# tier4/icp_rust

Hardware: AMD Instinct MI355X
Metric: ICP iterations/sec on 1M-pt 3D pair (higher is better)
Workload: dtype f64

## Files before the change

icp_rust_amd/csrc/nn_grid.hip:

```cpp
#include "common.hpp"
#include <type_traits>

namespace icp {

__device__ __forceinline__ int cell_coord(double v, double lo, double inv_h, int n) {
  double t = floor((v - lo) * inv_h);
  t = fmin(fmax(t, 0.), (double)(n - 1));
  return (int)t;
}

__global__ void k_grid_bbox(const double *__restrict__ dst, unsigned m, int dim, double *__restrict__ part) {
  __shared__ double smn[3][256], smx[3][256];
  double mn[3], mx[3];
  for (int d = 0; d < 3; ++d) {
    mn[d] = __builtin_huge_val();
    mx[d] = -__builtin_huge_val();
  }
  for (unsigned i = blockIdx.x * 256 + threadIdx.x; i < m; i += gridDim.x * 256)
    for (int d = 0; d < dim; ++d) {
      const double v = dst[(size_t)i * dim + d];
      mn[d] = fmin(mn[d], v);
      mx[d] = fmax(mx[d], v);
    }
  for (int d = 0; d < 3; ++d) {
// ... 799 lines not shown
    }
  };

  int iz = lo_c[2], iy = lo_c[1];
  float dz2 = (DIM == 3 && !wide) ? slab2(2, iz) : 0.f;
  for (;;) {
    uint32_t ra0 = 0, ra1 = 0, ra2 = 0, ra3 = 0, rz0 = 0, rz1 = 0, rz2 = 0, rz3 = 0;
    int nr = 0;
    while (nr < 4 && iz <= hi_c[2]) {
      if (iy > hi_c[1]) {
        iy = lo_c[1];
        ++iz;
        if (DIM == 3 && !wide && iz <= hi_c[2]) dz2 = slab2(2, iz);
        continue;
      }
      const int cy = iy++;
      int xl = lo_c[0], xh = hi_c[0];
      if (!wide) {
        const float dyz = slab2(1, cy) + dz2;
        if (dyz > bf) {
          if (CERT) skip2 = fminf(skip2, dyz);
          continue;
        }
        const float hw = __builtin_amdgcn_sqrtf(bf - dyz) * 1.000001f + mgf;
        xl = max(xl, cell_lo(qf[0] - hw, em[0], 0));
        xh = min(xh, cell_hi(qf[0] + hw, em[0], 0));
        if (xl > xh) {
          if (CERT) skip2 = 0.f;
          continue;
        }
        if (CERT) {
          if (xl > lo_c[0]) skip2 = fminf(skip2, slab2(0, xl - 1) + dyz);
          if (xh < hi_c[0]) skip2 = fminf(skip2, slab2(0, xh + 1) + dyz);
        }
      }
      const uint32_t rb = ((uint32_t)iz * g.n[1] + cy) * g.n[0];
      const uint32_t ra = rb + xl, rz = rb + xh + 1;
      if (nr == 0) ra0 = ra, rz0 = rz;
      else if (nr == 1) ra1 = ra, rz1 = rz;
      else if (nr == 2) ra2 = ra, rz2 = rz;
      else ra3 = ra, rz3 = rz;
      ++nr;
    }
    if (nr == 0) break;
    if (nr < 2) ra1 = ra0, rz1 = rz0;
    if (nr < 3) ra2 = ra0, rz2 = rz0;
    if (nr < 4) ra3 = ra0, rz3 = rz0;
    const uint32_t s0 = start[ra0], e0 = start[rz0];
    const uint32_t s1 = start[ra1], e1 = start[rz1];
    const uint32_t s2 = start[ra2], e2 = start[rz2];
    const uint32_t s3 = start[ra3], e3 = start[rz3];
    const uint32_t n0 = e0 > s0 ? (e0 - s0 + 3) >> 2 : 0u;
    const uint32_t n1 = (nr > 1 && e1 > s1) ? (e1 - s1 + 3) >> 2 : 0u;
    const uint32_t n2 = (nr > 2 && e2 > s2) ? (e2 - s2 + 3) >> 2 : 0u;
    const uint32_t n3 = (nr > 3 && e3 > s3) ? (e3 - s3 + 3) >> 2 : 0u;
    const uint32_t o1 = n0, o2 = o1 + n1, o3 = o2 + n2, Q = o3 + n3;
    const uint32_t d0 = s0, d1 = s1 - 4u * o1, d2 = s2 - 4u * o2, d3 = s3 - 4u * o3;
    constexpr uint32_t kQ = ICP_WARM_QUADS, kR = 4 * kQ;
    for (uint32_t base = 0; base < Q; base += kQ) {
      GridPoint t[kR];
      const uint4 *line[kQ];
#pragma unroll
      for (uint32_t h2 = 0; h2 < kQ; ++h2) {
        const uint32_t j = min(base + h2, Q - 1);
        uint32_t dq = d0;
        if (j >= o1) dq = d1;
        if (j >= o2) dq = d2;
        if (j >= o3) dq = d3;
        line[h2] = reinterpret_cast<const uint4 *>(pts) + (size_t)(uint32_t)(4u * j + dq);
      }
#pragma unroll
      for (uint32_t u = 0; u < kR; ++u) {
        const uint4 w = line[u >> 2][u & 3];
        t[u].x = __uint_as_float(w.x);
        t[u].y = __uint_as_float(w.y);
        t[u].z = __uint_as_float(w.z);
        t[u].idx = w.w;
      }
      __builtin_amdgcn_sched_barrier(0);
      float sc[kR];
#pragma unroll
      for (uint32_t u = 0; u < kR; ++u) {
        const float fx = qf[0] - t[u].x, fy = qf[1] - t[u].y;
        float s2 = __builtin_fmaf(fy, fy, fx * fx);
        if (DIM == 3) {
          const float fz = qf[2] - t[u].z;
          s2 = __builtin_fmaf(fz, fz, s2);
        }
        sc[u] = s2;
      }
#pragma unroll
      for (uint32_t u = 0; u < kR; ++u)
        if (!(sc[u] > thr32) && t[u].idx != bi) consider(t[u].idx);
      if (CERT) {
#pragma unroll
        for (uint32_t u = 0; u < kR; ++u) m2 = fminf(m2, t[u].idx != bi ? sc[u] : __builtin_huge_valf());
      }
    }
  }
  uint32_t cert_bits = 0;
  if (CERT && !wide && bi != 0xffffffffu) {
    const float seen = __builtin_amdgcn_sqrtf(m2) * 0.9999994f - ecf;
    const float skipped = __builtin_amdgcn_sqrtf(skip2) * 0.9999997f;
    const float cert = fminf(seen, skipped);
    const float abs_lo = (cert + (cd.r_lo * s_norm_lo + cd.t_lo) * 0.9999997f) * 0.9999997f;
    if (cert > 0.f && abs_lo > 0.f && abs_lo < __builtin_huge_valf()) cert_bits = __float_as_uint(abs_lo);
  }
  if (bi == 0xffffffffu) {
    bi = 0;
    bx = dst[0];
    by = dst[1];
    bz = DIM == 3 ? dst[2] : 0.;
  }
  if (CERT || SEEDED || bi != pm.idx) {
    PrevMatch out;
    out.x = bx;
    out.y = by;
    out.z = bz;
    out.idx = bi;
    out.pad = cert_bits;
    prev[k] = out;
  }
  if (idx) idx[i] = bi;
  if (a) a[i] = make_double2(q[0], q[1]);
  if (b) b[i] = make_double2(bx, by);
}

template <int DIM, bool CERT>
__global__ __launch_bounds__(kGridThreads) ICP_WARM_ATTR void k_nn_grid_warm(const double *__restrict__ src,
                                                               const uint32_t *__restrict__ perm, unsigned n, Pose T,
                                                               GridParams g, const uint32_t *__restrict__ start,
                                                               const GridPoint *__restrict__ pts,
                                                               const double *__restrict__ dst, uint32_t *__restrict__ idx,
                                                               double2 *__restrict__ a, double2 *__restrict__ b,
                                                               PrevMatch *prev, CertDecay cd, unsigned xcd_chunk) {
  const unsigned k = xcd_wave(blockIdx.x, gridDim.x, xcd_chunk) * kGridThreads + threadIdx.x;
  if (k >= n) return;
  warm_query<DIM, CERT>(k, src, perm, T, g, start, pts, dst, idx, a, b, prev, cd);
}

#ifndef ICP_COOP_ITEMS
#define ICP_COOP_ITEMS 2
#endif
#ifndef ICP_COOP_ROWS
#define ICP_COOP_ROWS 4
#endif
#ifndef ICP_COOP_FLUSH_AT
#define ICP_COOP_FLUSH_AT 96
#endif
constexpr int kCoopItems = ICP_COOP_ITEMS;
constexpr int kCoopRows = ICP_COOP_ROWS;
constexpr int kCoopCandCap = 256;
constexpr int kCoopFlushAt = ICP_COOP_FLUSH_AT;
struct CoopLds {
  uint32_t pref[64];
  uint32_t rows_d[64][kCoopRows];
  uint32_t rows_o[64][kCoopRows];
  float4 oq[64];
  uint32_t obi[64];
  uint2 cand[kCoopCandCap];
  unsigned long long fkey[64];
  uint32_t fidx[64];
  uint32_t fwin[64];
};

#ifdef ICP_COOP_PROFILE
__device__ unsigned long long g_coop_prof[64][12];
__device__ long long g_coop_span[16384][2];
__device__ unsigned long long g_coop_rows[32];
#define COOP_STAMP(i)                                                  \
  do {                                                                 \
    asm volatile("s_waitcnt vmcnt(0) lgkmcnt(0)" ::: "memory");        \
    const long long now_ = wall_clock64();                             \
    cprof[i] += (unsigned long long)(now_ - ct_last);                  \
    ct_last = now_;                                                    \
  } while (0)
#define COOP_COUNT(i, v) (cprof[i] += (v))
#else
#define COOP_STAMP(i) ((void)0)
#define COOP_COUNT(i, v) ((void)0)
#endif

template <int DIM, bool SEEDED>
__device__ __forceinline__ void warm_wave(const unsigned k, const unsigned n, const double *__restrict__ src,
                                          const uint32_t *__restrict__ perm, Pose T, const GridParams &g,
                                          const uint32_t *__restrict__ start, const GridPoint *__restrict__ pts,
                                          const double *__restrict__ dst, uint32_t *__restrict__ idx,
                                          double2 *__restrict__ a, double2 *__restrict__ b, PrevMatch *prev, PrevMatch seed,
                                          CoopLds &S) {
  const unsigned lane = threadIdx.x;
#ifdef ICP_COOP_PROFILE
  unsigned long long cprof[12] = {0, 0, 0, 0, 0, 0, 0, 1, 0, 0, 0, 0};
  long long ct_last = wall_clock64();
  const long long ct_first = ct_last;
#endif
  const bool in_range = k < n;
  const unsigned kk = in_range ? k : n - 1;
  const unsigned i = perm ? perm[kk] : kk;
  double q[3];
  q[0] = src[(size_t)kk * DIM + 0];
  q[1] = src[(size_t)kk * DIM + 1];
  q[2] = DIM == 3 ? src[(size_t)kk * DIM + 2] : 0.;
  {
    const double nx = (T.r00 * q[0] + T.r01 * q[1]) + T.tx;
    const double ny = (T.r10 * q[0] + T.r11 * q[1]) + T.ty;
    q[0] = nx;
    q[1] = ny;
  }
  const PrevMatch pm = SEEDED ? seed : prev[kk];
  const bool no_match = pm.idx == 0xffffffffu;
  bool alive = in_range && !no_match;
  auto dist2 = [&](double tx, double ty, double tz) -> double {
    const double ddx = q[0] - tx, ddy = q[1] - ty;
    double dd = ddx * ddx + ddy * ddy;
    if (DIM == 3) {
      const double ddz = q[2] - tz;
      dd = dd + ddz * ddz;
    }
    return dd;
  };
  double best = dist2(pm.x, pm.y, pm.z);
  uint32_t bi = pm.idx;
  double bx = pm.x, by = pm.y, bz = pm.z;
  if (!(best == best)) {
    best = __builtin_huge_val();
    bi = 0xffffffffu;
  }
  float qf[3], amax = 0.f;
#pragma unroll
  for (int d = 0; d < 3; ++d) {
    qf[d] = d < DIM ? (float)(q[d] - g.lo[d]) : 0.f;
    amax = fmaxf(amax, fabsf(qf[d]));
  }
  const float mgf = 4e-7f * (amax + g.ext);
  const float ecf = 2.1e-7f * (amax + g.ext);
  float bf, rf, thr32;
  auto set_radius = [&]() {
    bf = fmaxf((float)best * 1.0000003f, 1e-37f);
    const float rs = __builtin_amdgcn_sqrtf(bf) * 1.0000003f;
    rf = rs + mgf;
    thr32 = (rs + ecf) * (rs + ecf) * 1.000005f;
  };
  set_radius();
  const bool wide = !(amax + rf < 1e18f);
  if (wide) {
    bf = __builtin_huge_valf();
    thr32 = __builtin_huge_valf();
  }
  const float hf[3] = {g.hf[0], g.hf[1], g.hf[2]};
  const float ihf[3] = {g.ihf[0], g.ihf[1], g.ihf[2]};
  auto cell_lo = [&](float v, float em, int d) -> int {
    const float t = fminf(fmaxf(__builtin_floorf(v * ihf[d] - em), 0.f), g.nm1f[d]);
    return (int)t;
  };
  auto cell_hi = [&](float v, float em, int d) -> int {
    const float t = fminf(fmaxf(__builtin_floorf(v * ihf[d] + em), 0.f), g.nm1f[d]);
    return (int)t;
  };
  int lo_c[3] = {0, 0, 0}, hi_c[3] = {0, 0, 0};
  float em[3];
#pragma unroll
  for (int d = 0; d < DIM; ++d) {
    em[d] = (fabsf(qf[d]) + rf) * ihf[d] * 4e-7f + 1e-3f;
    lo_c[d] = wide ? 0 : cell_lo(qf[d] - rf, em[d], d);
    hi_c[d] = wide ? g.n[d] - 1 : cell_hi(qf[d] + rf, em[d], d);
  }
  auto slab2 = [&](int d, int c) -> float {
    const float e0 = (float)c * hf[d];
    const float below = c <= 0 ? -__builtin_huge_valf() : e0 - qf[d];
    const float above = c >= g.n[d] - 1 ? -__builtin_huge_valf() : qf[d] - (e0 + hf[d]);
    const float v = fmaxf(fmaxf(below, above) - mgf, 0.f);
    return v * v * 0.9999997f;
  };
  S.oq[lane] = make_float4(qf[0], qf[1], qf[2], thr32);
  S.obi[lane] = bi;
  S.fkey[lane] = 0x7ff0000000000000ull;
  S.fidx[lane] = 0xffffffffu;
  S.fwin[lane] = lane;
  COOP_STAMP(0);

  unsigned cnt = 0;
  auto flush = [&]() {
    COOP_COUNT(10, 1);
    COOP_COUNT(11, cnt);
    for (unsigned base = 0; base < cnt; base += 64) {
      const unsigned e = base + lane;
      const bool have = e < cnt;
      const uint2 c = S.cand[have ? e : base];
      const uint32_t ti = c.y;
      const double tx = dst[(size_t)ti * DIM + 0], ty = dst[(size_t)ti * DIM + 1];
      const double tz = DIM == 3 ? dst[(size_t)ti * DIM + 2] : 0.;
      const int sel = (int)(c.x << 2);
      double oqd[3];
#pragma unroll
      for (int d = 0; d < 3; ++d) {
        const unsigned lo = (unsigned)__builtin_amdgcn_ds_bpermute(sel, (int)__double2loint(q[d]));
        const unsigned hi = (unsigned)__builtin_amdgcn_ds_bpermute(sel, (int)__double2hiint(q[d]));
        oqd[d] = __hiloint2double((int)hi, (int)lo);
      }
      const double ddx = oqd[0] - tx, ddy = oqd[1] - ty;
      double dd = ddx * ddx + ddy * ddy;
      if (DIM == 3) {
        const double ddz = oqd[2] - tz;
        dd = dd + ddz * ddz;
      }
      const unsigned long long key = (unsigned long long)__double_as_longlong(dd);
      if (have) atomicMin(&S.fkey[c.x], key);
      __syncthreads();
      const bool first = have && S.fkey[c.x] == key;
      if (first) atomicMin(&S.fidx[c.x], ti);
      __syncthreads();
      if (first && S.fidx[c.x] == ti) S.fwin[c.x] = lane;
      __syncthreads();
      const double d2 = __longlong_as_double((long long)S.fkey[lane]);
      const uint32_t t2 = S.fidx[lane];
      const int wsel = (int)(S.fwin[lane] << 2);
      double wx[3];
      {
        const double tc[3] = {tx, ty, tz};
#pragma unroll
        for (int d = 0; d < 3; ++d) {
          const unsigned lo = (unsigned)__builtin_amdgcn_ds_bpermute(wsel, (int)__double2loint(tc[d]));
          const unsigned hi = (unsigned)__builtin_amdgcn_ds_bpermute(wsel, (int)__double2hiint(tc[d]));
          wx[d] = __hiloint2double((int)hi, (int)lo);
        }
      }
      if (d2 < best || (d2 == best && t2 < bi)) {
        best = d2;
        bi = t2;
        bx = wx[0];
        by = wx[1];
        bz = wx[2];
      }
      S.fkey[lane] = 0x7ff0000000000000ull;
      S.fidx[lane] = 0xffffffffu;
      S.fwin[lane] = lane;
      __syncthreads();
    }
    cnt = 0;
    if (!wide) set_radius();
    __syncthreads();
    S.oq[lane].w = thr32;
    S.obi[lane] = bi;
    __syncthreads();
  };

  int ty = lo_c[1], tz = lo_c[2];
  unsigned mask = 0;
  auto make_mask = [&](const bool on) {
    int ny = 1, nz = 1;
    if (__ballot(on && ty + 1 <= hi_c[1]) != 0ull) ny = 2;
    if (__ballot(on && ty + 2 <= hi_c[1]) != 0ull) ny = 4;
    if (DIM == 3) {
      if (__ballot(on && tz + 1 <= hi_c[2]) != 0ull) nz = 2;
      if (__ballot(on && tz + 2 <= hi_c[2]) != 0ull) nz = 4;
    }
    bool vy[4], vz[4];
    float sy[4], sz[4];
    unsigned m = 0;
    auto ey = [&](const int j) {
      vy[j] = ty + j <= hi_c[1];
      sy[j] = wide ? 0.f : slab2(1, ty + j);
    };
    auto ez = [&](const int j) {
      vz[j] = tz + j <= hi_c[2];
      sz[j] = (DIM == 3 && !wide) ? slab2(2, tz + j) : 0.f;
    };
    auto row = [&](const int jz) {
      auto bit = [&](const int jy) {
        if (vy[jy] && vz[jz] && !(sy[jy] + sz[jz] > bf)) m |= 1u << (jz * 4 + jy);
      };
      bit(0);
      if (ny > 1) bit(1);
      if (ny > 2) {
        bit(2);
        bit(3);
      }
    };
    ey(0);
    if (ny > 1) ey(1);
    if (ny > 2) {
      ey(2);
      ey(3);
    }
    ez(0);
    row(0);
    if (DIM == 3 && nz > 1) {
      ez(1);
      row(1);
      if (nz > 2) {
        ez(2);
        ez(3);
        row(2);
        row(3);
      }
    }
    if (on) mask = m;
  };
  make_mask(alive);
  const bool wave_tiles = __ballot(alive && (hi_c[1] - lo_c[1] >= 4 || hi_c[2] - lo_c[2] >= 4)) != 0ull;
#ifdef ICP_COOP_PROFILE
  unsigned rows_total = 0;
#endif
  for (;;) {
    int nr = 0;
    uint32_t rlo[kCoopRows], rhi[kCoopRows];
#pragma unroll
    for (int r = 0; r < kCoopRows; ++r) rlo[r] = rhi[r] = 0u;
    auto pick = [&](const bool on, uint32_t &d, uint32_t &o) -> bool {
      const bool take = on && mask != 0u;
      const int r = __ffs((int)mask) - 1;
      if (on) mask &= mask - 1u;
      const int jy = r & 3, jz = r >> 2;
      const uint32_t rb = ((uint32_t)(tz + jz) * g.n[1] + (uint32_t)(ty + jy)) * g.n[0];
      if (take) {
        d = rb + lo_c[0];
        o = rb + hi_c[0] + 1;
      }
      return take;
    };
#pragma unroll
    for (int r = 0; r < kCoopRows; ++r) {
      if (__ballot(mask != 0u) == 0ull) break;
      nr += pick(true, rlo[r], rhi[r]) ? 1 : 0;
    }
    if (wave_tiles)
      for (bool need = alive && nr < kCoopRows; __ballot(need) != 0ull; need = alive && nr < kCoopRows) {
        const bool adv = need && mask == 0u;
        if (adv) {
          ty += 4;
          if (ty > hi_c[1]) {
            ty = lo_c[1];
            tz += 4;
          }
          if (tz > hi_c[2]) alive = false;
        }
        if (__ballot(adv && alive) != 0ull) make_mask(adv && alive);
        const bool more = need && !adv;
        if (__ballot(more) != 0ull) {
          uint32_t d = 0u, o = 0u;
          const bool take = pick(more, d, o);
#pragma unroll
          for (int r = 0; r < kCoopRows; ++r)
            if (take && nr == r) {
              rlo[r] = d;
              rhi[r] = o;
            }
          nr += take ? 1 : 0;
        }
      }
    if (__ballot(nr > 0) == 0ull) break;
#ifdef ICP_COOP_PROFILE
    rows_total += (unsigned)nr;
#endif
    COOP_STAMP(1);
    COOP_COUNT(8, 1);
    uint32_t sb[kCoopRows], se[kCoopRows];
#pragma unroll
    for (int r = 0; r < kCoopRows; ++r) {
      sb[r] = start[rlo[r]];
      se[r] = start[rhi[r]];
    }
    uint32_t rd[kCoopRows], ro[kCoopRows], Q = 0;
#pragma unroll
    for (int r = 0; r < kCoopRows; ++r) {
      const uint32_t nq = ((nr > r) & (se[r] > sb[r])) ? ((se[r] - sb[r] + 3) >> 2) : 0u;
      ro[r] = Q;
      rd[r] = sb[r] - 4u * Q;
      Q += nq;
    }
    COOP_STAMP(2);
    uint32_t incl = Q;
#define ICP_SCAN_DPP(v, ctrl, rows) (uint32_t)__builtin_amdgcn_update_dpp(0, (int)(v), ctrl, rows, 0xf, true)
    incl += ICP_SCAN_DPP(incl, 0x111, 0xf);
    incl += ICP_SCAN_DPP(incl, 0x112, 0xf);
    incl += ICP_SCAN_DPP(incl, 0x114, 0xf);
    incl += ICP_SCAN_DPP(incl, 0x118, 0xf);
    incl += ICP_SCAN_DPP(incl, 0x142, 0xa);
    incl += ICP_SCAN_DPP(incl, 0x143, 0xc);
#undef ICP_SCAN_DPP
    const uint32_t total = (uint32_t)__builtin_amdgcn_readlane((int)incl, 63);
    S.pref[lane] = incl - Q;
#pragma unroll
    for (int r = 0; r < kCoopRows; ++r) {
      S.rows_d[lane][r] = rd[r];
      S.rows_o[lane][r] = ro[r];
    }
    __syncthreads();
    COOP_STAMP(3);
    auto batch = [&](auto ni_, const uint32_t w0) {
      constexpr int NI = decltype(ni_)::value;
      COOP_COUNT(9, 1);
      GridPoint t[4 * NI];
      unsigned own[NI];
      bool has[NI];
#pragma unroll
      for (int it = 0; it < NI; ++it) {
        const uint32_t w = w0 + 64u * it + lane;
        has[it] = w < total;
        const uint32_t wc = has[it] ? w : total - 1;
        unsigned L = 0;
#pragma unroll
        for (unsigned st = 32; st >= 1; st >>= 1)
          if (S.pref[L + st] <= wc) L += st;
        own[it] = L;
        const uint32_t j = wc - S.pref[L];
        uint32_t dq = S.rows_d[L][0];
#pragma unroll
        for (int r = 1; r < kCoopRows; ++r)
          if (j >= S.rows_o[L][r]) dq = S.rows_d[L][r];
        const uint4 *line = reinterpret_cast<const uint4 *>(pts) + (size_t)(uint32_t)(4u * j + dq);
#pragma unroll
        for (int u = 0; u < 4; ++u) {
          const uint4 wv = line[u];
          t[4 * it + u].x = __uint_as_float(wv.x);
          t[4 * it + u].y = __uint_as_float(wv.y);
          t[4 * it + u].z = __uint_as_float(wv.z);
          t[4 * it + u].idx = wv.w;
        }
      }
      __builtin_amdgcn_sched_barrier(0);
#pragma unroll
      for (int it = 0; it < NI; ++it) {
        const float4 oq = S.oq[own[it]];
        const uint32_t obi = S.obi[own[it]];
        bool pass[4];
        unsigned long long bal[4];
        unsigned fresh = 0;
#pragma unroll
        for (int u = 0; u < 4; ++u) {
          const float fx = oq.x - t[4 * it + u].x, fy = oq.y - t[4 * it + u].y;
          float s2 = __builtin_fmaf(fy, fy, fx * fx);
          if (DIM == 3) {
            const float fz = oq.z - t[4 * it + u].z;
            s2 = __builtin_fmaf(fz, fz, s2);
          }
          pass[u] = has[it] & !(s2 > oq.w) & (t[4 * it + u].idx != obi);
          bal[u] = __ballot(pass[u]);
          fresh += (unsigned)__popcll(bal[u]);
        }
        if (fresh == 0) continue;
        if (cnt + fresh > (unsigned)kCoopCandCap) flush();
        const unsigned long long below = (1ull << lane) - 1ull;
#pragma unroll
        for (int u = 0; u < 4; ++u) {
          if (pass[u]) S.cand[cnt + (unsigned)__popcll(bal[u] & below)] = make_uint2(own[it], t[4 * it + u].idx);
          cnt += (unsigned)__popcll(bal[u]);
        }
      }
    };
    {
      uint32_t w0 = 0;
      for (; w0 + 64u < total; w0 += 64u * kCoopItems) batch(std::integral_constant<int, kCoopItems>{}, w0);
      if (w0 < total) batch(std::integral_constant<int, 1>{}, w0);
    }
    __syncthreads();
    COOP_STAMP(4);
    if (cnt >= (unsigned)kCoopFlushAt) {
      flush();
      COOP_STAMP(5);
    }
  }
  COOP_STAMP(1);
  if (cnt > 0) flush();
  COOP_STAMP(5);
#ifdef ICP_COOP_PROFILE
  auto coop_report = [&]() {
    asm volatile("s_waitcnt vmcnt(0) lgkmcnt(0)" ::: "memory");
    cprof[6] += (unsigned long long)(wall_clock64() - ct_last);
    if (in_range) atomicAdd(&g_coop_rows[rows_total < 31u ? rows_total : 31u], 1ull);
    if (lane == 0) {
      for (int j = 0; j < 12; ++j) atomicAdd(&g_coop_prof[blockIdx.x & 63][j], cprof[j]);
      if (blockIdx.x < 16384u) {
        g_coop_span[blockIdx.x][0] = ct_first;
        g_coop_span[blockIdx.x][1] = wall_clock64();
      }
    }
  };
#endif

  auto emit = [&]() {
    if (!in_range) return;
    if (no_match) {
      if (SEEDED) prev[k] = pm;
      if (idx) idx[i] = 0;
      if (a) a[i] = make_double2(q[0], q[1]);
      if (b) b[i] = make_double2(dst[0], dst[1]);
      return;
    }
    if (bi == 0xffffffffu) {
      bi = 0;
      bx = dst[0];
      by = dst[1];
      bz = DIM == 3 ? dst[2] : 0.;
    }
    if (SEEDED || bi != pm.idx) {
      PrevMatch out;
      out.x = bx;
      out.y = by;
      out.z = bz;
      out.idx = bi;
      out.pad = 0;
      prev[k] = out;
    }
    if (idx) idx[i] = bi;
    if (a) a[i] = make_double2(q[0], q[1]);
    if (b) b[i] = make_double2(bx, by);
  };
  emit();
#ifdef ICP_COOP_PROFILE
  coop_report();
#endif
}

#ifdef ICP_COOP_WAVES
#define ICP_COOP_ATTR __attribute__((amdgpu_waves_per_eu(ICP_COOP_WAVES, ICP_COOP_WAVES)))
#else
#define ICP_COOP_ATTR
#endif
template <int DIM>
__global__ __launch_bounds__(kGridThreads) ICP_COOP_ATTR void k_nn_grid_warm_coop(const double *__restrict__ src,
                                                                    const uint32_t *__restrict__ perm, unsigned n, Pose T,
                                                                    GridParams g, const uint32_t *__restrict__ start,
                                                                    const GridPoint *__restrict__ pts,
                                                                    const double *__restrict__ dst, uint32_t *__restrict__ idx,
                                                                    double2 *__restrict__ a, double2 *__restrict__ b,
                                                                    PrevMatch *prev, unsigned xcd_chunk,
                                                                    const AheadPose *__restrict__ ahead) {
  __shared__ CoopLds S;
  if (ahead) {
    if (!ahead->valid) return;
    T = ahead->T;
  }
  const unsigned k = xcd_wave(blockIdx.x, gridDim.x, xcd_chunk) * kGridThreads + threadIdx.x;
  warm_wave<DIM, false>(k, n, src, perm, T, g, start, pts, dst, idx, a, b, prev, PrevMatch{0., 0., 0., 0xffffffffu, 0u}, S);
}

constexpr int kCertLists = 16;
constexpr int kCertCtrStride = 32;
constexpr int kCertThreads = 256;

template <int DIM>
__global__ __launch_bounds__(kCertThreads) void k_nn_cert(const double *__restrict__ src,
                                                          const uint32_t *__restrict__ perm, unsigned n, Pose T,
                                                          const double *__restrict__ dst, uint32_t *__restrict__ idx,
                                                          double2 *__restrict__ a, double2 *__restrict__ b,
                                                          const PrevMatch *__restrict__ prev, CertDecay cd,
                                                          uint32_t *__restrict__ lists, unsigned list_cap,
                                                          unsigned *ctr, unsigned *ctr_next) {
  __shared__ unsigned s_cnt[kCertThreads / 64], s_base;
  const unsigned k = blockIdx.x * kCertThreads + threadIdx.x;
  const int lane = threadIdx.x & 63, wave = threadIdx.x >> 6;
  if (blockIdx.x == 0 && threadIdx.x < kCertLists) ctr_next[threadIdx.x * kCertCtrStride] = 0;
  bool fail = false;
  if (k < n) {
    const unsigned i = perm ? perm[k] : k;
    double q[3];
    q[0] = src[(size_t)k * DIM + 0];
    q[1] = src[(size_t)k * DIM + 1];
    q[2] = DIM == 3 ? src[(size_t)k * DIM + 2] : 0.;
    const PrevMatch pm = prev[k];
    const float s_norm = __builtin_amdgcn_sqrtf((float)(q[0] * q[0] + q[1] * q[1]) * 1.0000003f) * 1.0000003f;
    {
      const double nx = (T.r00 * q[0] + T.r01 * q[1]) + T.tx;
      const double ny = (T.r10 * q[0] + T.r11 * q[1]) + T.ty;
      q[0] = nx;
      q[1] = ny;
    }
    if (pm.idx == 0xffffffffu) {
      if (idx) idx[i] = 0;
      if (a) a[i] = make_double2(q[0], q[1]);
      if (b) b[i] = make_double2(dst[0], dst[1]);
    } else {
      const double ddx = q[0] - pm.x, ddy = q[1] - pm.y;
      double best = ddx * ddx + ddy * ddy;
      if (DIM == 3) {
        const double ddz = q[2] - pm.z;
        best = best + ddz * ddz;
      }
      const float bf = fmaxf((float)best * 1.0000003f, 1e-37f);
      const float rs = __builtin_amdgcn_sqrtf(bf) * 1.0000003f;
      const float moved = (cd.r_hi * s_norm + cd.t_hi) * 1.000001f;
      const float c_abs = __uint_as_float(pm.pad);
      const bool pass = pm.pad != 0u && (rs + moved) * 1.000001f < c_abs;
      if (pass) {
        if (idx) idx[i] = pm.idx;
        if (a) a[i] = make_double2(q[0], q[1]);
        if (b) b[i] = make_double2(pm.x, pm.y);
      } else {
        fail = true;
      }
    }
  }
  const unsigned long long mask = __ballot(fail);
  if (lane == 0) s_cnt[wave] = (unsigned)__popcll(mask);
  __syncthreads();
  const int list = blockIdx.x % kCertLists;
  if (threadIdx.x == 0) {
    unsigned tot = 0;
#pragma unroll
    for (int w = 0; w < kCertThreads / 64; ++w) tot += s_cnt[w];
    s_base = tot ? atomicAdd(&ctr[list * kCertCtrStride], tot) : 0u;
  }
  __syncthreads();
  if (fail) {
    unsigned pos = s_base + (unsigned)__popcll(mask & ((1ull << lane) - 1ull));
#pragma unroll
    for (int w = 0; w < kCertThreads / 64; ++w) pos += w < wave ? s_cnt[w] : 0u;
    if (pos < list_cap) lists[(size_t)list * list_cap + pos] = k;
  }
}

template <int DIM>
__global__ __launch_bounds__(kGridThreads) ICP_WARM_ATTR void k_nn_walk_lists(
    const double *__restrict__ src, const uint32_t *__restrict__ perm, Pose T, GridParams g,
    const uint32_t *__restrict__ start, const GridPoint *__restrict__ pts, const double *__restrict__ dst,
    uint32_t *__restrict__ idx, double2 *__restrict__ a, double2 *__restrict__ b, PrevMatch *prev, CertDecay cd,
    const uint32_t *__restrict__ lists, unsigned list_cap, const unsigned *__restrict__ ctr) {
  const unsigned cnt = min(ctr[blockIdx.y * kCertCtrStride], list_cap);
  const unsigned j = blockIdx.x * kGridThreads + threadIdx.x;
  if (j >= cnt) return;
  const unsigned k = lists[(size_t)blockIdx.y * list_cap + j];
  warm_query<DIM, true>(k, src, perm, T, g, start, pts, dst, idx, a, b, prev, cd);
}


template <int DIM>
__device__ __forceinline__ PrevMatch seed_match(const unsigned k, const double *__restrict__ src, const Pose &T,
                                                 const GridParams &g, const uint32_t *__restrict__ start,
                                                 const GridPoint *__restrict__ pts, const double *__restrict__ dst) {
  double q[3];
  q[0] = src[(size_t)k * DIM + 0];
  q[1] = src[(size_t)k * DIM + 1];
  q[2] = DIM == 3 ? src[(size_t)k * DIM + 2] : 0.;
  {
    const double nx = (T.r00 * q[0] + T.r01 * q[1]) + T.tx;
    const double ny = (T.r10 * q[0] + T.r11 * q[1]) + T.ty;
    q[0] = nx;
    q[1] = ny;
  }
  PrevMatch out;
  out.x = out.y = out.z = 0.;
  out.idx = 0xffffffffu;
  out.pad = 0;
  const bool finite = fabs(q[0]) <= 1.7976931348623157e308 && fabs(q[1]) <= 1.7976931348623157e308 &&
                      (DIM < 3 || fabs(q[2]) <= 1.7976931348623157e308);
  if (finite) {
    float qf[3] = {0.f, 0.f, 0.f};
    int c[3] = {0, 0, 0};
#pragma unroll
    for (int d = 0; d < DIM; ++d) {
      qf[d] = (float)(q[d] - g.lo[d]);
      c[d] = (int)fminf(fmaxf(__builtin_floorf(qf[d] * (float)g.inv_h[d]), 0.f), (float)(g.n[d] - 1));
    }
    constexpr int kSeedDiv = 4;
    constexpr uint32_t kSeedBatch = 8;
    const int hx = g.fx > kSeedDiv ? g.fx / kSeedDiv : 1;
    float best = __builtin_huge_valf();
    uint32_t bi = 0xffffffffu, any = 0xffffffffu;
    for (int r = 0;; ++r) {
      const int wx = r * g.fx + hx;
      const int x0 = max(c[0] - wx, 0), x1 = min(c[0] + wx, g.n[0] - 1);
      const int y0 = max(c[1] - r, 0), y1 = min(c[1] + r, g.n[1] - 1);
      const int z0 = DIM == 3 ? max(c[2] - r, 0) : 0, z1 = DIM == 3 ? min(c[2] + r, g.n[2] - 1) : 0;
      for (int iz = z0; iz <= z1; ++iz)
        for (int iy = y0; iy <= y1; ++iy) {
          const uint32_t rb = ((uint32_t)iz * g.n[1] + iy) * g.n[0];
          const uint32_t s0 = start[rb + x0], e0 = start[rb + x1 + 1];
          for (uint32_t j0 = s0; j0 < e0; j0 += kSeedBatch) {
            uint4 wv[kSeedBatch];
#pragma unroll
            for (uint32_t u = 0; u < kSeedBatch; ++u) wv[u] = reinterpret_cast<const uint4 *>(pts)[min(j0 + u, e0 - 1)];
#pragma unroll
            for (uint32_t u = 0; u < kSeedBatch; ++u) {
              const uint4 w = wv[u];
              const float fx = qf[0] - __uint_as_float(w.x), fy = qf[1] - __uint_as_float(w.y);
              const float fz = DIM == 3 ? qf[2] - __uint_as_float(w.z) : 0.f;
              const float s2 = fx * fx + fy * fy + fz * fz;
              if (s2 < best) {
                best = s2;
                bi = w.w;
              } else if (s2 == __builtin_huge_valf() && any == 0xffffffffu && fabsf(__uint_as_float(w.x)) < __builtin_huge_valf() &&
                         fabsf(__uint_as_float(w.y)) < __builtin_huge_valf() && fabsf(__uint_as_float(w.z)) < __builtin_huge_valf()) {
                any = w.w;
              }
            }
          }
        }
      if (bi != 0xffffffffu || any != 0xffffffffu) break;
      if (x0 == 0 && x1 == g.n[0] - 1 && y0 == 0 && y1 == g.n[1] - 1 && z0 == 0 && z1 == (DIM == 3 ? g.n[2] - 1 : 0)) break;
    }
    if (bi == 0xffffffffu) bi = any;
    if (bi != 0xffffffffu) {
      out.x = dst[(size_t)bi * DIM + 0];
      out.y = dst[(size_t)bi * DIM + 1];
      out.z = DIM == 3 ? dst[(size_t)bi * DIM + 2] : 0.;
      out.idx = bi;
    }
  }
  return out;
}

template <int DIM>
__global__ __launch_bounds__(kGridThreads) void k_nn_grid_seeded(const double *__restrict__ src,
                                                                 const uint32_t *__restrict__ perm, unsigned n, Pose T,
                                                                 GridParams g, const uint32_t *__restrict__ start,
                                                                 const GridPoint *__restrict__ pts,
                                                                 const double *__restrict__ dst, uint32_t *__restrict__ idx,
                                                                 double2 *__restrict__ a, double2 *__restrict__ b,
                                                                 PrevMatch *prev) {
  __shared__ CoopLds S;
  const unsigned k = xcd_wave(blockIdx.x, gridDim.x, kXcdChunk) * kGridThreads + threadIdx.x;
  const PrevMatch pm = seed_match<DIM>(k < n ? k : n - 1, src, T, g, start, pts, dst);
  warm_wave<DIM, true>(k, n, src, perm, T, g, start, pts, dst, idx, a, b, prev, pm, S);
}

__global__ void k_query_cell(const double *__restrict__ src, unsigned n, int dim, Pose T, GridParams g, int blk,
                             uint32_t *__restrict__ cell_of, int xshift) {
  const unsigned i = blockIdx.x * blockDim.x + threadIdx.x;
  if (i >= n) return;
  double q[3] = {src[(size_t)i * dim], src[(size_t)i * dim + 1], dim == 3 ? src[(size_t)i * dim + 2] : 0.};
  const double nx = (T.r00 * q[0] + T.r01 * q[1]) + T.tx;
  const double ny = (T.r10 * q[0] + T.r11 * q[1]) + T.ty;
  q[0] = nx;
  q[1] = ny;
  int c[3] = {0, 0, 0};
  for (int d = 0; d < dim; ++d) c[d] = cell_coord(q[d], g.lo[d], g.inv_h[d], g.n[d]);
  c[0] >>= xshift;
  const uint32_t nxk = ((uint32_t)g.n[0] + (1u << xshift) - 1u) >> xshift;
  const uint32_t nyb = ((uint32_t)g.n[1] + (1u << blk) - 1) >> blk, m = (1u << blk) - 1;
  const uint32_t brow = ((uint32_t)c[2] >> blk) * nyb + ((uint32_t)c[1] >> blk);
  const uint32_t sub = (((uint32_t)c[2] & m) << blk) | ((uint32_t)c[1] & m);
  cell_of[i] = ((brow * nxk + (uint32_t)c[0]) << (2 * blk)) | sub;
}

__global__ void k_query_gather(const double *__restrict__ src, unsigned n, int dim, const uint32_t *__restrict__ perm,
                               double *__restrict__ sorted) {
  const size_t c = (size_t)blockIdx.x * blockDim.x + threadIdx.x;
  const size_t tot = (size_t)n * dim;
  const size_t e0 = 2 * c, e1 = e0 + 1;
  if (e0 >= tot) return;
  const size_t k0 = e0 / (unsigned)dim, k1 = e1 / (unsigned)dim;
  const double v0 = src[(size_t)perm[k0] * dim + (e0 - k0 * dim)];
  if (e1 < tot) {
    const double v1 = src[(size_t)perm[k1] * dim + (e1 - k1 * dim)];
    reinterpret_cast<double2 *>(sorted)[c] = make_double2(v0, v1);
  } else {
    sorted[e0] = v0;
  }
}

__global__ void k_unpermute_idx(const uint32_t *__restrict__ slot_idx, const uint32_t *__restrict__ perm, unsigned n,
                                uint32_t *__restrict__ out) {
  const unsigned k = blockIdx.x * blockDim.x + threadIdx.x;
  if (k < n) out[perm[k]] = slot_idx[k];
}

hipError_t launch_unpermute_idx(icp_handle *h, const uint32_t *d_slot_idx, size_t n, uint32_t *d_out) {
  if (n == 0) return hipSuccess;
  hipLaunchKernelGGL(k_unpermute_idx, dim3(((unsigned)n + 255) / 256), dim3(256), 0, h->stream, d_slot_idx,
                     (const uint32_t *)h->qsort.d_perm, (unsigned)n, d_out);
  return hipGetLastError();
}

hipError_t prepare_queries(icp_handle *h, const double *d_src, size_t n_, const Pose &T) {
  Grid &G = h->grid;
  QuerySort &Q = h->qsort;
  Q.valid = false;
  Q.fold_n = 0;
  if (!G.built || n_ == 0) return hipSuccess;
  const unsigned n = (unsigned)n_;
  hipError_t e;
  hipStream_t s = h->stream;
  if (n_ > Q.cap) {
    if ((e = hipStreamSynchronize(s)) != hipSuccess) return e;
    (void)hipFree(Q.d_cell_of);
    (void)hipFree(Q.d_perm);
    (void)hipFree(Q.d_sorted);
    (void)hipFree(Q.d_prev);
    (void)hipFree(Q.d_cert_lists);
    (void)hipFree(Q.d_cert_ctr);
    Q.last_cert_ctr = nullptr;
    Q.d_prev = nullptr;
    Q.d_cert_lists = nullptr;
    Q.d_cert_ctr = nullptr;
    Q.d_cell_of = Q.d_perm = nullptr;
    Q.d_sorted = nullptr;
    Q.cap = 0;
    Q.fold_n = 0;
    if ((e = hipMalloc(&Q.d_cell_of, n_ * 4)) != hipSuccess) return e;
    if ((e = hipMalloc(&Q.d_perm, n_ * 4)) != hipSuccess) return e;
    if ((e = hipMalloc(&Q.d_sorted, n_ * 3 * sizeof(double))) != hipSuccess) return e;
    if ((e = hipMalloc(&Q.d_prev, n_ * sizeof(PrevMatch))) != hipSuccess) return e;
    if ((e = hipMalloc(&Q.d_cert_lists, (n_ + (size_t)(kCertLists + 1) * kCertThreads) * sizeof(uint32_t))) != hipSuccess) return e;
    if ((e = hipMalloc(&Q.d_cert_ctr, (size_t)2 * kCertLists * kCertCtrStride * sizeof(unsigned))) != hipSuccess) return e;
    if ((e = hipMemsetAsync(Q.d_cert_ctr, 0, (size_t)2 * kCertLists * kCertCtrStride * sizeof(unsigned), s)) != hipSuccess) return e;
    Q.cert_seq = 0;
    Q.cap = n_;
  }
  Q.identity = (long)n <= kGridCoopMaxN || Q.presorted;
  Q.presorted = false;
  if (Q.identity) {
    Q.have_prev = false;
    Q.have_certs = false;
    Q.have_pose = Q.have_pose_before = false;
    Q.decay_r = Q.decay_t = 0.;
    Q.src = d_src;
    Q.n = n_;
    Q.valid = true;
    return hipSuccess;
  }
  const unsigned long long keys = (unsigned long long)G.p.n[2] * (unsigned long long)G.p.n[1] * (unsigned long long)G.p.n[0];
  hipLaunchKernelGGL(k_query_cell, dim3((n + 255) / 256), dim3(256), 0, s, d_src, n, h->dim, T, G.p, 0, Q.d_cell_of, 0);
  unsigned bits = 1;
  while (bits < 32 && (1ull << bits) < keys) ++bits;
  if ((e = stable_sort_cells(Q.d_cell_of, Q.d_perm, n, bits, Q.d_tmp, Q.cap_tmp, s)) != hipSuccess) return e;
  if (Q.sort_only) {
    Q.sort_only = false;
    Q.src = d_src;
    Q.n = n_;
    return hipGetLastError();
  }
  {
    const size_t pairs = ((size_t)n * h->dim + 1) / 2;
    hipLaunchKernelGGL(k_query_gather, dim3((unsigned)((pairs + 255) / 256)), dim3(256), 0, s, d_src, n, h->dim,
                       (const uint32_t *)Q.d_perm, Q.d_sorted);
  }
  Q.have_prev = false;
  Q.have_certs = false;
  Q.have_pose = Q.have_pose_before = false;
  Q.decay_r = Q.decay_t = 0.;
  if ((e = hipGetLastError()) != hipSuccess) return e;
  Q.src = d_src;
  Q.n = n_;
  Q.valid = true;
  return hipSuccess;
}

hipError_t launch_nn_grid_ahead(icp_handle *h, const double *d_src, size_t n_, const AheadPose *d_pose, double *d_a,
                                double *d_b, uint32_t *d_idx, bool *launched) {
  *launched = false;
  const Grid &G = h->grid;
  QuerySort &Q = h->qsort;
  if (n_ == 0 || n_ >= 0xffffffffull || !d_pose || h->m == 0 || !G.built || !G.p.f32_ok) return hipSuccess;
  const unsigned n = (unsigned)n_;
  if (!(Q.valid && Q.src == d_src && Q.n == n_ && Q.have_prev)) return hipSuccess;
  const bool coop = (long)n <= kGridCoopMaxN;
  const double *q_src = !Q.identity ? Q.d_sorted : d_src;
  const uint32_t *q_perm = (!Q.slot_order && !Q.identity) ? Q.d_perm : nullptr;
  hipEvent_t ev0 = nullptr, ev1 = nullptr;
  if (h->profile > 0 && (h->prof_seen++ % (unsigned)h->profile) == 0) {
    if (!h->prof_free.empty()) {
      ev0 = h->prof_free.back().first;
      ev1 = h->prof_free.back().second;
      h->prof_free.pop_back();
      (void)hipEventRecord(ev0, h->stream);
    } else if (hipEventCreate(&ev0) == hipSuccess && hipEventCreate(&ev1) == hipSuccess)
      (void)hipEventRecord(ev0, h->stream);
  }
  const unsigned blocks = (unsigned)(((size_t)n * (coop ? 4 : 1) + kGridThreads - 1) / kGridThreads);
  Q.have_pose = false;
  Q.have_certs = false;
  if (coop) {
    if (h->dim == 3)
      hipLaunchKernelGGL((k_nn_grid<3, true, false, 4>), dim3(blocks), dim3(kGridThreads), 0, h->stream, q_src, q_perm, n,
                         transform_identity(), G.p, G.d_start, G.d_pts, h->d_dst, d_idx, (double2 *)d_a, (double2 *)d_b,
                         (const PrevMatch *)Q.d_prev, Q.d_prev, d_pose);
// ... 202 lines not shown
```

Before: 10160.

## Trim cooperative NN wave's LDS and register footprint for higher occupancy

Shrinks the per-wave shared-memory struct by dropping the prefix, owner-best-index and winner arrays. Candidate entries are split into a 32-bit target array and a byte owner array, and the prefix and best index are read across lanes with ds_bpermute instead of LDS. The winner's coordinates are written into shared memory only when they improve the match, which removes one barrier and six bpermutes per flush. Several values (the permuted index, best coordinates, box bounds and the radius-squared term) are recomputed or packed so fewer registers stay live, and a static_assert pins the LDS size to 24 one-wave groups per CU. The intent is more resident waves and less synchronisation, at the cost of extra recomputation and cross-lane shuffles.

```diff
diff --git a/icp_rust_amd/csrc/nn_grid.hip b/icp_rust_amd/csrc/nn_grid.hip
--- a/icp_rust_amd/csrc/nn_grid.hip
+++ b/icp_rust_amd/csrc/nn_grid.hip
@@ -975,17 +975,20 @@
 constexpr int kCoopRows = ICP_COOP_ROWS;
 constexpr int kCoopCandCap = 256;
 constexpr int kCoopFlushAt = ICP_COOP_FLUSH_AT;
+constexpr unsigned kLdsPerCu = 160u * 1024u, kLdsGranule = 1280u, kCoopGroupsPerCu = 24u;
 struct CoopLds {
-  uint32_t pref[64];
   uint32_t rows_d[64][kCoopRows];
-  uint32_t rows_o[64][kCoopRows];
+  uint32_t rows_o[64][kCoopRows - 1];
   float4 oq[64];
-  uint32_t obi[64];
-  uint2 cand[kCoopCandCap];
+  uint32_t cand_t[kCoopCandCap];
+  uint8_t cand_o[kCoopCandCap];
   unsigned long long fkey[64];
   uint32_t fidx[64];
-  uint32_t fwin[64];
+  double win[3][64];
 };
+
+static_assert((sizeof(CoopLds) + kLdsGranule - 1) / kLdsGranule * kLdsGranule * kCoopGroupsPerCu <= kLdsPerCu,
+              "CoopLds: 24 one-wave workgroups per CU no longer fit the LDS (six waves per SIMD)");
 
 #ifdef ICP_COOP_PROFILE
 __device__ unsigned long long g_coop_prof[64][12];
@@ -1005,13 +1008,14 @@
 #endif
 
 template <int DIM, bool SEEDED>
-__device__ __forceinline__ void warm_wave(const unsigned k, const unsigned n, const double *__restrict__ src,
+__device__ __forceinline__ void warm_wave(const unsigned kbase, const unsigned n, const double *__restrict__ src,
                                           const uint32_t *__restrict__ perm, Pose T, const GridParams &g,
                                           const uint32_t *__restrict__ start, const GridPoint *__restrict__ pts,
                                           const double *__restrict__ dst, uint32_t *__restrict__ idx,
                                           double2 *__restrict__ a, double2 *__restrict__ b, PrevMatch *prev, PrevMatch seed,
                                           CoopLds &S) {
   const unsigned lane = threadIdx.x;
+  const unsigned k = kbase + lane;
 #ifdef ICP_COOP_PROFILE
   unsigned long long cprof[12] = {0, 0, 0, 0, 0, 0, 0, 1, 0, 0, 0, 0};
   long long ct_last = wall_clock64();
@@ -1019,7 +1023,6 @@
 #endif
   const bool in_range = k < n;
   const unsigned kk = in_range ? k : n - 1;
-  const unsigned i = perm ? perm[kk] : kk;
   double q[3];
   q[0] = src[(size_t)kk * DIM + 0];
   q[1] = src[(size_t)kk * DIM + 1];
@@ -1044,7 +1047,6 @@
   };
   double best = dist2(pm.x, pm.y, pm.z);
   uint32_t bi = pm.idx;
-  double bx = pm.x, by = pm.y, bz = pm.z;
   if (!(best == best)) {
     best = __builtin_huge_val();
     bi = 0xffffffffu;
@@ -1057,19 +1059,16 @@
   }
   const float mgf = 4e-7f * (amax + g.ext);
   const float ecf = 2.1e-7f * (amax + g.ext);
-  float bf, rf, thr32;
-  auto set_radius = [&]() {
-    bf = fmaxf((float)best * 1.0000003f, 1e-37f);
-    const float rs = __builtin_amdgcn_sqrtf(bf) * 1.0000003f;
-    rf = rs + mgf;
-    thr32 = (rs + ecf) * (rs + ecf) * 1.000005f;
-  };
-  set_radius();
+  float thr32;
+  auto radius2 = [&]() -> float { return fmaxf((float)best * 1.0000003f, 1e-37f); };
+  auto set_radius = [&](const float ec) -> float {
+    const float rs = __builtin_amdgcn_sqrtf(radius2()) * 1.0000003f;
+    thr32 = (rs + ec) * (rs + ec) * 1.000005f;
+    return rs;
+  };
+  const float rf = set_radius(ecf) + mgf;
   const bool wide = !(amax + rf < 1e18f);
-  if (wide) {
-    bf = __builtin_huge_valf();
-    thr32 = __builtin_huge_valf();
-  }
+  if (wide) thr32 = __builtin_huge_valf();
   const float hf[3] = {g.hf[0], g.hf[1], g.hf[2]};
   const float ihf[3] = {g.ihf[0], g.ihf[1], g.ihf[2]};
   auto cell_lo = [&](float v, float em, int d) -> int {
@@ -1088,18 +1087,21 @@
     lo_c[d] = wide ? 0 : cell_lo(qf[d] - rf, em[d], d);
     hi_c[d] = wide ? g.n[d] - 1 : cell_hi(qf[d] + rf, em[d], d);
   }
-  auto slab2 = [&](int d, int c) -> float {
+  auto slab2 = [&](int d, int c, const float qd, const float mg) -> float {
     const float e0 = (float)c * hf[d];
-    const float below = c <= 0 ? -__builtin_huge_valf() : e0 - qf[d];
-    const float above = c >= g.n[d] - 1 ? -__builtin_huge_valf() : qf[d] - (e0 + hf[d]);
-    const float v = fmaxf(fmaxf(below, above) - mgf, 0.f);
+    const float below = c <= 0 ? -__builtin_huge_valf() : e0 - qd;
+    const float above = c >= g.n[d] - 1 ? -__builtin_huge_valf() : qd - (e0 + hf[d]);
+    const float v = fmaxf(fmaxf(below, above) - mg, 0.f);
     return v * v * 0.9999997f;
   };
+  const uint32_t ybox = (uint32_t)lo_c[1] | ((uint32_t)hi_c[1] << 16), zbox = (uint32_t)lo_c[2] | ((uint32_t)hi_c[2] << 16);
+  const int xlo = lo_c[0], xhi = hi_c[0];
   S.oq[lane] = make_float4(qf[0], qf[1], qf[2], thr32);
-  S.obi[lane] = bi;
   S.fkey[lane] = 0x7ff0000000000000ull;
   S.fidx[lane] = 0xffffffffu;
-  S.fwin[lane] = lane;
+  S.win[0][lane] = pm.x;
+  S.win[1][lane] = pm.y;
+  S.win[2][lane] = pm.z;
   COOP_STAMP(0);
 
   unsigned cnt = 0;
@@ -1109,11 +1111,11 @@
     for (unsigned base = 0; base < cnt; base += 64) {
       const unsigned e = base + lane;
       const bool have = e < cnt;
-      const uint2 c = S.cand[have ? e : base];
-      const uint32_t ti = c.y;
+      const uint32_t ti = S.cand_t[have ? e : base];
+      const unsigned co = S.cand_o[have ? e : base];
       const double tx = dst[(size_t)ti * DIM + 0], ty = dst[(size_t)ti * DIM + 1];
       const double tz = DIM == 3 ? dst[(size_t)ti * DIM + 2] : 0.;
-      const int sel = (int)(c.x << 2);
+      const int sel = (int)(co << 2);
       double oqd[3];
 #pragma unroll
       for (int d = 0; d < 3; ++d) {
@@ -1128,66 +1130,62 @@
         dd = dd + ddz * ddz;
       }
       const unsigned long long key = (unsigned long long)__double_as_longlong(dd);
-      if (have) atomicMin(&S.fkey[c.x], key);
+      if (have) atomicMin(&S.fkey[co], key);
       __syncthreads();
-      const bool first = have && S.fkey[c.x] == key;
-      if (first) atomicMin(&S.fidx[c.x], ti);
+      const bool first = have && S.fkey[co] == key;
+      if (first) atomicMin(&S.fidx[co], ti);
       __syncthreads();
-      if (first && S.fidx[c.x] == ti) S.fwin[c.x] = lane;
-      __syncthreads();
+      const bool won = first && S.fidx[co] == ti;
       const double d2 = __longlong_as_double((long long)S.fkey[lane]);
       const uint32_t t2 = S.fidx[lane];
-      const int wsel = (int)(S.fwin[lane] << 2);
-      double wx[3];
-      {
-        const double tc[3] = {tx, ty, tz};
-#pragma unroll
-        for (int d = 0; d < 3; ++d) {
-          const unsigned lo = (unsigned)__builtin_amdgcn_ds_bpermute(wsel, (int)__double2loint(tc[d]));
-          const unsigned hi = (unsigned)__builtin_amdgcn_ds_bpermute(wsel, (int)__double2hiint(tc[d]));
-          wx[d] = __hiloint2double((int)hi, (int)lo);
-        }
-      }
-      if (d2 < best || (d2 == best && t2 < bi)) {
+      const bool upd = d2 < best || (d2 == best && t2 < bi);
+      if (upd) {
         best = d2;
         bi = t2;
-        bx = wx[0];
-        by = wx[1];
-        bz = wx[2];
+      }
+      const unsigned long long takes = __ballot(upd);
+      if (won && ((takes >> co) & 1ull) != 0ull) {
+        S.win[0][co] = tx;
+        S.win[1][co] = ty;
+        S.win[2][co] = tz;
       }
       S.fkey[lane] = 0x7ff0000000000000ull;
       S.fidx[lane] = 0xffffffffu;
-      S.fwin[lane] = lane;
       __syncthreads();
     }
     cnt = 0;
-    if (!wide) set_radius();
+    if (!wide) set_radius(ecf);
     __syncthreads();
     S.oq[lane].w = thr32;
-    S.obi[lane] = bi;
     __syncthreads();
   };
 
   int ty = lo_c[1], tz = lo_c[2];
   unsigned mask = 0;
   auto make_mask = [&](const bool on) {
+    uint32_t yb = ybox, zb = zbox;
+    asm volatile("" : "+v"(yb), "+v"(zb));
+    const int hi_y = (int)(yb >> 16), hi_z = (int)(zb >> 16);
+    const float4 me = S.oq[lane];
+    const float mg = 4e-7f * (fmaxf(fmaxf(fabsf(me.x), fabsf(me.y)), fabsf(me.z)) + g.ext);
+    const float bf = wide ? __builtin_huge_valf() : radius2();
     int ny = 1, nz = 1;
-    if (__ballot(on && ty + 1 <= hi_c[1]) != 0ull) ny = 2;
-    if (__ballot(on && ty + 2 <= hi_c[1]) != 0ull) ny = 4;
+    if (__ballot(on && ty + 1 <= hi_y) != 0ull) ny = 2;
+    if (__ballot(on && ty + 2 <= hi_y) != 0ull) ny = 4;
     if (DIM == 3) {
-      if (__ballot(on && tz + 1 <= hi_c[2]) != 0ull) nz = 2;
-      if (__ballot(on && tz + 2 <= hi_c[2]) != 0ull) nz = 4;
+      if (__ballot(on && tz + 1 <= hi_z) != 0ull) nz = 2;
+      if (__ballot(on && tz + 2 <= hi_z) != 0ull) nz = 4;
     }
     bool vy[4], vz[4];
     float sy[4], sz[4];
     unsigned m = 0;
     auto ey = [&](const int j) {
-      vy[j] = ty + j <= hi_c[1];
-      sy[j] = wide ? 0.f : slab2(1, ty + j);
+      vy[j] = ty + j <= hi_y;
+      sy[j] = wide ? 0.f : slab2(1, ty + j, me.y, mg);
     };
     auto ez = [&](const int j) {
-      vz[j] = tz + j <= hi_c[2];
-      sz[j] = (DIM == 3 && !wide) ? slab2(2, tz + j) : 0.f;
+      vz[j] = tz + j <= hi_z;
+      sz[j] = (DIM == 3 && !wide) ? slab2(2, tz + j, me.z, mg) : 0.f;
     };
     auto row = [&](const int jz) {
       auto bit = [&](const int jy) {
@@ -1237,8 +1235,8 @@
       const int jy = r & 3, jz = r >> 2;
       const uint32_t rb = ((uint32_t)(tz + jz) * g.n[1] + (uint32_t)(ty + jy)) * g.n[0];
       if (take) {
-        d = rb + lo_c[0];
-        o = rb + hi_c[0] + 1;
+        d = rb + xlo;
+        o = rb + xhi + 1;
       }
       return take;
     };
@@ -1251,12 +1249,14 @@
       for (bool need = alive && nr < kCoopRows; __ballot(need) != 0ull; need = alive && nr < kCoopRows) {
         const bool adv = need && mask == 0u;
         if (adv) {
+          uint32_t yb = ybox, zb = zbox;
+          asm volatile("" : "+v"(yb), "+v"(zb));
           ty += 4;
-          if (ty > hi_c[1]) {
-            ty = lo_c[1];
+          if (ty > (int)(yb >> 16)) {
+            ty = (int)(yb & 0xffffu);
             tz += 4;
           }
-          if (tz > hi_c[2]) alive = false;
+          if (tz > (int)(zb >> 16)) alive = false;
         }
         if (__ballot(adv && alive) != 0ull) make_mask(adv && alive);
         const bool more = need && !adv;
@@ -1303,11 +1303,11 @@
     incl += ICP_SCAN_DPP(incl, 0x143, 0xc);
 #undef ICP_SCAN_DPP
     const uint32_t total = (uint32_t)__builtin_amdgcn_readlane((int)incl, 63);
-    S.pref[lane] = incl - Q;
+    const int excl = (int)(incl - Q);
 #pragma unroll
     for (int r = 0; r < kCoopRows; ++r) {
       S.rows_d[lane][r] = rd[r];
-      S.rows_o[lane][r] = ro[r];
+      if (r > 0) S.rows_o[lane][r - 1] = ro[r];
     }
     __syncthreads();
     COOP_STAMP(3);
@@ -1325,13 +1325,13 @@
         unsigned L = 0;
 #pragma unroll
         for (unsigned st = 32; st >= 1; st >>= 1)
-          if (S.pref[L + st] <= wc) L += st;
+          if ((uint32_t)__builtin_amdgcn_ds_bpermute((int)((L + st) << 2), excl) <= wc) L += st;
         own[it] = L;
-        const uint32_t j = wc - S.pref[L];
+        const uint32_t j = wc - (uint32_t)__builtin_amdgcn_ds_bpermute((int)(L << 2), excl);
         uint32_t dq = S.rows_d[L][0];
 #pragma unroll
         for (int r = 1; r < kCoopRows; ++r)
-          if (j >= S.rows_o[L][r]) dq = S.rows_d[L][r];
+          if (j >= S.rows_o[L][r - 1]) dq = S.rows_d[L][r];
         const uint4 *line = reinterpret_cast<const uint4 *>(pts) + (size_t)(uint32_t)(4u * j + dq);
 #pragma unroll
         for (int u = 0; u < 4; ++u) {
@@ -1346,7 +1346,7 @@
 #pragma unroll
       for (int it = 0; it < NI; ++it) {
         const float4 oq = S.oq[own[it]];
-        const uint32_t obi = S.obi[own[it]];
+        const uint32_t obi = (uint32_t)__builtin_amdgcn_ds_bpermute((int)(own[it] << 2), (int)bi);
         bool pass[4];
         unsigned long long bal[4];
         unsigned fresh = 0;
@@ -1367,7 +1367,11 @@
         const unsigned long long below = (1ull << lane) - 1ull;
 #pragma unroll
         for (int u = 0; u < 4; ++u) {
-          if (pass[u]) S.cand[cnt + (unsigned)__popcll(bal[u] & below)] = make_uint2(own[it], t[4 * it + u].idx);
+          if (pass[u]) {
+            const unsigned at = cnt + (unsigned)__popcll(bal[u] & below);
+            S.cand_t[at] = t[4 * it + u].idx;
+            S.cand_o[at] = (uint8_t)own[it];
+          }
           cnt += (unsigned)__popcll(bal[u]);
         }
       }
@@ -1404,6 +1408,10 @@
 
   auto emit = [&]() {
     if (!in_range) return;
+    unsigned l2 = lane;
+    asm volatile("" : "+v"(l2));
+    const unsigned k = kbase + l2;
+    const unsigned i = perm ? perm[k] : k;
     if (no_match) {
       if (SEEDED) prev[k] = pm;
       if (idx) idx[i] = 0;
@@ -1411,6 +1419,8 @@
       if (b) b[i] = make_double2(dst[0], dst[1]);
       return;
     }
+    double bx = S.win[0][lane], by = S.win[1][lane], bz = S.win[2][lane];
+    asm volatile("" : "+v"(bx), "+v"(by), "+v"(bz));
     if (bi == 0xffffffffu) {
       bi = 0;
       bx = dst[0];
@@ -1455,8 +1465,8 @@
     if (!ahead->valid) return;
     T = ahead->T;
   }
-  const unsigned k = xcd_wave(blockIdx.x, gridDim.x, xcd_chunk) * kGridThreads + threadIdx.x;
-  warm_wave<DIM, false>(k, n, src, perm, T, g, start, pts, dst, idx, a, b, prev, PrevMatch{0., 0., 0., 0xffffffffu, 0u}, S);
+  const unsigned kb = xcd_wave(blockIdx.x, gridDim.x, xcd_chunk) * kGridThreads;
+  warm_wave<DIM, false>(kb, n, src, perm, T, g, start, pts, dst, idx, a, b, prev, PrevMatch{0., 0., 0., 0xffffffffu, 0u}, S);
 }
 
 constexpr int kCertLists = 16;
@@ -1633,9 +1643,9 @@
                                                                  double2 *__restrict__ a, double2 *__restrict__ b,
                                                                  PrevMatch *prev) {
   __shared__ CoopLds S;
-  const unsigned k = xcd_wave(blockIdx.x, gridDim.x, kXcdChunk) * kGridThreads + threadIdx.x;
+  const unsigned kb = xcd_wave(blockIdx.x, gridDim.x, kXcdChunk) * kGridThreads, k = kb + threadIdx.x;
   const PrevMatch pm = seed_match<DIM>(k < n ? k : n - 1, src, T, g, start, pts, dst);
-  warm_wave<DIM, true>(k, n, src, perm, T, g, start, pts, dst, idx, a, b, prev, pm, S);
+  warm_wave<DIM, true>(kb, n, src, perm, T, g, start, pts, dst, idx, a, b, prev, pm, S);
 }
 
 __global__ void k_query_cell(const double *__restrict__ src, unsigned n, int dim, Pose T, GridParams g, int blk,
```

After: 10140. About the same (-0.2%).
